# cloneofsimo/paint-with-words-sd

Hardware: AMD Instinct MI355X
Metric: 512x512 images/sec (30 steps, CFG) SD1.5+PwW (higher is better)
Workload: dtype bf16

## Files before the change

### include/pww_hip.h

```cpp
#ifndef PWW_HIP_H
#define PWW_HIP_H

#include <stddef.h>
#include <stdint.h>

#ifdef __cplusplus
extern "C" {
#endif

#define PWW_VERSION 126

#define PWW_OK 0
#define PWW_EINVAL (-22)
#define PWW_ENOTSUP (-95)
#define PWW_EHIP (-5)

#define PWW_DTYPE_F16 0
#define PWW_DTYPE_BF16 1

#define PWW_MAX_HEAD_DIM 160

typedef struct pww_attn_desc {
    int32_t dtype;
    int32_t B, H, N, M, D;
// ... 55 lines not shown
    int64_t k_stride[2];
} pww_qproj_desc_t;

int pww_qproj_stat(const void *x, const void *w, void *q, const void *k, const float *gate, const pww_qproj_desc_t *desc,
                   int32_t stat_kind, double *partials, size_t partials_bytes, void *stream);
int32_t pww_qproj_parts(const pww_qproj_desc_t *desc);

int pww_cross_attn_fwd_parts(const void *q, const void *k, const void *v, void *o, const float *bias, int32_t stat_kind,
                             float coeff_scalar, const float *gate, const pww_attn_desc_t *desc, const double *partials,
                             int32_t nparts, double *stats_out, const pww_cross_opts_t *opts, void *stream);

int pww_qk_parts(const void *q, const void *k, const float *gate, const pww_attn_desc_t *desc, int32_t stat_kind, int32_t gated_images,
                 double *partials, size_t partials_bytes, void *stream);
int32_t pww_qk_parts_count(const pww_attn_desc_t *desc);

#define PWW_LAYOUT_NCHW 0
#define PWW_LAYOUT_NHWC 1
#define PWW_ACT_NONE 0
#define PWW_ACT_SILU 1
typedef struct pww_gn_desc {
    int32_t dtype;
    int32_t layout;
    int32_t B, C, HW, G;
    float eps;
    int32_t act;
    int32_t add_stride;
    int32_t _pad;
} pww_gn_desc_t;

size_t pww_group_norm_workspace_bytes(const pww_gn_desc_t *desc);
int pww_group_norm_fwd(const void *x, const void *pre_c, const void *add_bc, const void *gamma, const void *beta, void *y,
                       const pww_gn_desc_t *desc, void *workspace, size_t workspace_bytes, void *stream);

typedef struct pww_ln_desc {
    int32_t dtype;
    int32_t C;
    int64_t rows;
    int64_t a_stride, x_stride, s_stride, y_stride;
    float eps;
    int32_t _pad;
} pww_ln_desc_t;
int pww_add_layer_norm(const void *a, const void *x, const void *gamma, const void *beta, void *s, void *y, const pww_ln_desc_t *desc, void *stream);
int pww_add_layer_norm_bias(const void *a, const void *x, const void *gamma, const void *beta, const void *post_bias, void *s, void *y,
                            const pww_ln_desc_t *desc, void *stream);
int pww_geglu(const void *h, void *y, int64_t rows, int32_t D, int64_t h_stride, int64_t y_stride, int32_t dtype, void *stream);
int pww_bias_residual(const void *r, const void *v, const void *bias, void *y, int32_t B, int32_t C, int32_t HW, int32_t layout, int32_t dtype, void *stream);

typedef struct pww_conv_desc {
    uint32_t size;
    int32_t dtype;
    int32_t B, Hin, Win, Cin, Cout;
    int32_t stride, upsample;
    int32_t tile_n, splitk;
    int32_t _pad;
} pww_conv_desc_t;
size_t pww_conv3x3_workspace_bytes(const pww_conv_desc_t *desc);
int pww_conv3x3_fwd(const void *x, const void *w, const void *bias, const void *residual, void *y, const pww_conv_desc_t *desc, void *workspace,
                    size_t workspace_bytes, void *stream);

typedef struct pww_probs_desc {
    uint32_t size;
    int32_t  images;
    int32_t  accumulate;
    float    weight;
    int64_t  out_stride[2];
} pww_probs_desc_t;

int pww_cross_attn_probs(const void *q, const void *k, const float *bias,
                         const double *stats, int32_t stat_kind, double stat_count, float coeff_scalar,
                         const float *gate, const pww_attn_desc_t *desc, const pww_cross_opts_t *opts,
                         float *out, const pww_probs_desc_t *pdesc, void *stream);

int pww_qk_reduce(const void *q, const void *k, const pww_attn_desc_t *desc,
                  double *stats, void *workspace, size_t workspace_bytes, void *stream);

typedef struct pww_region {
    uint8_t r, g, b, _pad;
    float strength;
} pww_region_t;

int pww_mask_build(const uint8_t *rgb, int32_t H, int32_t W,
                   const pww_region_t *regions, int32_t R,
                   const int32_t *col_ptr, const int32_t *col_reg, int32_t T,
                   float *out8, float *out16, float *out32, float *out64, void *stream);

int pww_mask_build_rgb(const uint8_t *rgb, int32_t H, int32_t W,
                       const pww_region_t *regions, int32_t R,
                       const int32_t *col_ptr, const int32_t *col_reg, int32_t T,
                       int32_t ratio, float *out, void *stream);

int pww_mask_build_f32(const float *masks, int32_t H, int32_t W, int32_t R,
                       const int32_t *col_ptr, const int32_t *col_reg, int32_t T,
                       int32_t ratio, float *out, void *stream);

int pww_mask_build_f32_levels(const float *masks, int32_t H, int32_t W, int32_t R, const int32_t *col_ptr, const int32_t *col_reg,
                              int32_t T, float *out8, float *out16, float *out32, float *out64, void *stream);

int pww_resize_tokens(const float *orig, int32_t H, int32_t W, int32_t T, int32_t oh, int32_t ow,
                      int32_t n_tokens, float *out, void *stream);

int pww_gauss_blur(const float *in, float *out, int32_t H, int32_t W, const float *weights, int32_t ksize,
                   double *tmp, void *stream);

int pww_inpaint_prep(const uint8_t *rgb, const uint8_t *mask, int32_t H, int32_t W, int32_t h, int32_t w,
                     float *mask_out, float *masked_image, float *mask_lat, void *stream);

int pww_cfg_combine(const void *cond, const void *uncond, float guidance, float *out,
// ... 39 lines not shown
```

### paint-with-words-sd_amd/build.py

```python
import os
import subprocess
import sys

HERE = os.path.dirname(os.path.abspath(__file__))
REPO = os.path.dirname(HERE)
CSRC = os.path.join(HERE, "csrc")
LIB = os.path.join(HERE, "pww_hip", "libpww_hip.so")
LIB_EXPERIMENTS = os.path.join(HERE, "pww_hip", "libpww_hip_experiments.so")
UNITS = [("pww_api.hip", [], ""), ("pww_attn.hip", [], ""), ("pww_cross.hip", [], ""), ("pww_cross_lean.hip", [], ""), ("pww_reduce.hip", [], ""),
         ("pww_mask.hip", [], ""), ("pww_qproj.hip", [], ""), ("pww_norm.hip", [], ""), ("pww_blocks.hip", [], ""), ("pww_conv.hip", [], ""), ("pww_probs.hip", [], ""),
         ("pww_attn_inst.hip", ["-DPWW_INST_F16"], ".f16"), ("pww_attn_inst.hip", ["-DPWW_INST_BF16"], ".bf16"),
         ("pww_cross_inst.hip", ["-DPWW_INST_F16", "-DPWW_INST_NW=2"], ".f16.nw2"), ("pww_cross_inst.hip", ["-DPWW_INST_F16", "-DPWW_INST_NW=4"], ".f16.nw4"),
         ("pww_cross_inst.hip", ["-DPWW_INST_BF16", "-DPWW_INST_NW=2"], ".bf16.nw2"), ("pww_cross_inst.hip", ["-DPWW_INST_BF16", "-DPWW_INST_NW=4"], ".bf16.nw4")]
EXPERIMENT_UNITS = [("pww_cross_out.hip", [], "")]
_ATTN_HEADERS = ["pww_tile.h", "pww_attn_core.h", "pww_cross_tile.h"]
SIDE_FLAGS = ["-fvisibility=hidden"]
SIDE_LIBS = {
    "long": ("pww_long.hip", _ATTN_HEADERS, "the long-prompt launches"),
    "scope": ("pww_scope.hip", _ATTN_HEADERS, "cross-attention with per-head / per-row score statistics"),
    "linear": ("pww_linear.hip", [], "linear layers with a bias / residual / GEGLU epilogue"),
    "regions": ("pww_regions.hip", [], "region masks and the per-pixel blend of the noise predictions"),
}
SOURCES = sorted({u[0] for u in UNITS + EXPERIMENT_UNITS})
HEADERS = ["pww_common.h", "pww_tile.h", "pww_attn_core.h", "pww_attn_kernel.h", "pww_cross_tile.h", "pww_cross_kernel.h", os.path.join(REPO, "include", "pww_hip.h")]
LIB_LONG, LIB_SCOPE, LIB_LINEAR, LIB_REGIONS = (os.path.join(HERE, "pww_hip", "libpww_hip_%s.so" % n) for n in SIDE_LIBS)
LONG_UNITS, SCOPE_UNITS, LINEAR_UNITS, REGIONS_UNITS = ([(v[0], SIDE_FLAGS, "")] for v in SIDE_LIBS.values())
HIPCC = os.environ.get("HIPCC", "/opt/rocm/bin/hipcc")
FLAGS = ["--offload-arch=gfx950", "-O3", "-std=c++17", "-fPIC", "-Wall",
         "-Wno-unused-function", "-mllvm", "-amdgpu-kernarg-preload-count=16"]


PER_FILE_FLAGS = {"pww_mask.hip": ["-ffp-contract=off"], "pww_regions.hip": ["-ffp-contract=off"]}


def _newer(target, deps):
    if not os.path.exists(target):
        return True
    t = os.path.getmtime(target)
    return any(os.path.getmtime(d) > t for d in deps)


def _deps():
    return ([os.path.join(CSRC, s) for s in SOURCES] + [h if os.path.isabs(h) else os.path.join(CSRC, h) for h in HEADERS] + [__file__])


def _build(lib, units, defines, objdir, verbose, jobs=None):
    os.makedirs(objdir, exist_ok=True)
    order = sorted(units, key=lambda u: {"pww_cross_inst.hip": 0, "pww_attn_inst.hip": 1, "pww_cross_lean.hip": 2}.get(u[0], 3))
    jobs = jobs or max(2, min(len(order), os.cpu_count() or 4, int(os.environ.get("MAX_JOBS", 16))))
    pending, running, objs = list(order), [], []
    while pending or running:
        while pending and len(running) < jobs:
            src, defs, suffix = pending.pop(0)
            o = os.path.join(objdir, src + suffix + ".o")
            objs.append(o)
            cmd = [HIPCC] + FLAGS + defines + defs + PER_FILE_FLAGS.get(src, []) + ["-c", os.path.join(CSRC, src), "-o", o]
            if verbose:
                print(" ".join(cmd))
            running.append((cmd, subprocess.Popen(cmd, stdout=subprocess.PIPE, stderr=subprocess.STDOUT, text=True)))
        cmd, p = running.pop(0)
        out, _ = p.communicate()
        if p.returncode != 0:
            for _, q in running:
                q.kill()
            raise RuntimeError("hipcc failed: %s\n%s" % (" ".join(cmd), out))
        if verbose and out.strip():
            print(out)
    subprocess.run([HIPCC, "--offload-arch=gfx950", "-shared", "-fPIC", "-s"] + sorted(objs) + ["-o", lib], check=True)
    return lib


def build_lib(force=False, verbose=False):
    if not force and not _newer(LIB, _deps()):
        return LIB
    return _build(LIB, UNITS, [], os.path.join(HERE, "build"), verbose)


# ... 49 lines not shown
```

### paint-with-words-sd_amd/csrc/pww_conv.hip

```cpp
#include "pww_common.h"

namespace pww {

namespace {

constexpr int CV_BM = 128, CV_THREADS = 256;
constexpr int CV_PF = 2;

__device__ __forceinline__ f32x4 mfma16(f16x8 a, f16x8 b, f32x4 c) { return __builtin_amdgcn_mfma_f32_16x16x32_f16(a, b, c, 0, 0, 0); }
__device__ __forceinline__ f32x4 mfma16(bf16x8 a, bf16x8 b, f32x4 c) { return __builtin_amdgcn_mfma_f32_16x16x32_bf16(a, b, c, 0, 0, 0); }

struct ConvCold {
    const void *bias, *residual;
    int nsplit, nslab;
};

__device__ __forceinline__ int xcd_remap(int orig, int nwg) {
    const int xcd = orig & 7, q = nwg >> 3, r = nwg & 7;
    return (xcd < r ? xcd * (q + 1) : r * (q + 1) + (xcd - r) * q) + (orig >> 3);
}

template <typename T>
__device__ __forceinline__ void epilogue4(const f32x4 &a, const ConvCold &cold, T *y, long off, int n) {
    typedef typename Vec<T>::v4 V4;
    V4 o;
#pragma unroll
    for (int j = 0; j < 4; ++j) o[j] = (T)a[j];
    if (cold.bias) {
        const V4 b = *reinterpret_cast<const V4 *>(reinterpret_cast<const T *>(cold.bias) + n);
#pragma unroll
        for (int j = 0; j < 4; ++j) o[j] = (T)((float)o[j] + (float)b[j]);
    }
    if (cold.residual) {
        const V4 r = *reinterpret_cast<const V4 *>(reinterpret_cast<const T *>(cold.residual) + off);
#pragma unroll
        for (int j = 0; j < 4; ++j) o[j] = (T)((float)r[j] + (float)o[j]);
    }
    *reinterpret_cast<V4 *>(y + off) = o;
}

template <typename T, int BN>
__global__ void __launch_bounds__(CV_THREADS, 2) conv3x3_kernel(const T *__restrict__ x, const T *__restrict__ w, void *__restrict__ out, int M, int N,
                                                            int Cin, int Hin, int Win, int Wo, int HWo, const ConvCold cold) {
    typedef typename Vec<T>::v8 V8;
    constexpr int BM = CV_BM, PF = CV_PF, XL = BM * 8 / CV_THREADS, WL = BN * 8 / CV_THREADS, RM = 4, RN = BN / 32;
    constexpr int XBYTES = BM * 128, STAGE = (BM + BN) * 128;
    __shared__ __attribute__((aligned(16))) char lds[2 * STAGE];

    const int geo = cold.nslab >> 24;
    const int nslab = cold.nslab & 0xffffff;
    const int stride = geo & 15, up = geo >> 4;
    const int Hv = Hin << up, Wv = Win << up;
    const int tid = threadIdx.x, lane = tid & 63, wave = tid >> 6, wm = wave >> 1, wn = wave & 1;
    const int ntm = (M + BM - 1) / BM;
    const int bid = xcd_remap(blockIdx.x, gridDim.x);
    const bool split = cold.nsplit > 1;
    const int tile = bid / cold.nsplit, ks = bid - tile * cold.nsplit;
    const int tm = tile % ntm, tn = tile / ntm;
    const int s_begin = (int)((long)ks * nslab / cold.nsplit), s_end = (int)((long)(ks + 1) * nslab / cold.nsplit);
    const int K9 = 9 * Cin;

    const int c = tid & 7;
    int pix[XL], y0[XL], x0[XL];
#pragma unroll
    for (int i = 0; i < XL; ++i) {
        int m = tm * BM + (tid >> 3) + 32 * i;
        m = m < M ? m : M - 1;
        const int b = m / HWo, rem = m - b * HWo, oy = rem / Wo, ox = rem - oy * Wo;
        pix[i] = b * Hin * Win;
        y0[i] = oy * stride - 1;
        x0[i] = ox * stride - 1;
    }
    const T *wrow = w + (long)(tn * BN + (tid >> 3)) * K9 + c * 8;
    const int swz = ((c ^ ((tid >> 3) & 7)) << 4);

    u32x4 xr[PF][XL], wr[PF][WL];
    unsigned xok[PF];
    int tap = s_begin / (Cin >> 6), ci0 = (s_begin - tap * (Cin >> 6)) << 6;
    const T *wnext = wrow + s_begin * 64;
    auto load = [&](int p) {
        const int ky = tap / 3, kx = tap - ky * 3;
        xok[p] = 0;
#pragma unroll
        for (int i = 0; i < XL; ++i) {
            const int iyv = y0[i] + ky, ixv = x0[i] + kx;
            const bool ok = (unsigned)iyv < (unsigned)Hv && (unsigned)ixv < (unsigned)Wv;
            const int iy = ok ? iyv >> up : 0, ix = ok ? ixv >> up : 0;
            xr[p][i] = *reinterpret_cast<const u32x4 *>(x + (unsigned)((pix[i] + iy * Win + ix) * Cin + ci0 + c * 8));
            xok[p] |= (unsigned)ok << i;
        }
#pragma unroll
        for (int j = 0; j < WL; ++j) wr[p][j] = *reinterpret_cast<const u32x4 *>(wnext + (long)(32 * j) * K9);
        wnext += 64;
        ci0 += 64;
        if (ci0 == Cin) { ci0 = 0; ++tap; }
    };
    auto store = [&](int p, int buf) {
        char *base = lds + buf * STAGE;
#pragma unroll
        for (int i = 0; i < XL; ++i) {
            const u32x4 z = {0u, 0u, 0u, 0u};
            *reinterpret_cast<u32x4 *>(base + ((tid >> 3) + 32 * i) * 128 + swz) = (xok[p] >> i) & 1u ? xr[p][i] : z;
        }
#pragma unroll
        for (int j = 0; j < WL; ++j) *reinterpret_cast<u32x4 *>(base + XBYTES + ((tid >> 3) + 32 * j) * 128 + swz) = wr[p][j];
    };

    f32x4 acc[RN][RM];
#pragma unroll
    for (int r = 0; r < RN; ++r)
#pragma unroll
        for (int i = 0; i < RM; ++i) acc[r][i] = f32x4{0.f, 0.f, 0.f, 0.f};

    const int fr = lane & 15, fq = lane >> 4;
    auto compute = [&](int buf) {
        const char *bx = lds + buf * STAGE, *bw = bx + XBYTES;
#pragma unroll
        for (int kk = 0; kk < 2; ++kk) {
            V8 xf[RM], wf[RN];
#pragma unroll
            for (int q = 0; q < RM; ++q) {
                const int row = wm * 64 + q * 16 + fr;
                xf[q] = *reinterpret_cast<const V8 *>(bx + row * 128 + (((kk * 4 + fq) ^ (row & 7)) << 4));
            }
#pragma unroll
            for (int r = 0; r < RN; ++r) {
                const int row = wn * (BN / 2) + r * 16 + fr;
                wf[r] = *reinterpret_cast<const V8 *>(bw + row * 128 + (((kk * 4 + fq) ^ (row & 7)) << 4));
            }
#pragma unroll
            for (int r = 0; r < RN; ++r)
#pragma unroll
                for (int q = 0; q < RM; ++q) acc[r][q] = mfma16(wf[r], xf[q], acc[r][q]);
        }
    };

    const int n = s_end - s_begin;
    load(0);
#pragma unroll
    for (int p = 1; p < PF; ++p)
        if (p < n) load(p);
    store(0, 0);
    __syncthreads();
    int i = 0;
    for (; i + 2 * PF <= n; i += PF) {
#pragma unroll
        for (int p = 0; p < PF; ++p) {
            load(p);
            compute((i + p) & 1);
            store((p + 1) % PF, (i + p + 1) & 1);
            __syncthreads();
        }
    }
#pragma unroll
    for (int t = 0; t < 2 * PF - 1; ++t) {
        if (i + t < n) {
            if (i + t + PF < n) load(t % PF);
            compute((i + t) & 1);
            if (i + t + 1 < n) store((t + 1) % PF, (i + t + 1) & 1);
            __syncthreads();
        }
    }

#pragma unroll
    for (int i = 0; i < RM; ++i) {
        const int m = tm * BM + wm * 64 + i * 16 + fr;
        if (m >= M) continue;
#pragma unroll
        for (int r = 0; r < RN; ++r) {
            const int n = tn * BN + wn * (BN / 2) + r * 16 + fq * 4;
            if (split) *reinterpret_cast<f32x4 *>(reinterpret_cast<float *>(out) + ((long)ks * M + m) * N + n) = acc[r][i];
            else epilogue4<T>(acc[r][i], cold, reinterpret_cast<T *>(out), (long)m * N + n, n);
        }
    }
}

template <typename T>
__global__ void __launch_bounds__(256) conv3x3_fold_kernel(const float *__restrict__ ws, T *__restrict__ y, long n4, int N, long MN, const ConvCold cold) {
    const long q = (long)blockIdx.x * 256 + threadIdx.x;
    if (q >= n4) return;
    const long off = q * 4;
    f32x4 a = *reinterpret_cast<const f32x4 *>(ws + off);
    for (int s = 1; s < cold.nsplit; ++s) a += *reinterpret_cast<const f32x4 *>(ws + s * MN + off);
    epilogue4<T>(a, cold, y, off, (int)(off % N));
}

struct ConvTune { int M, N, nslab, bn, nsplit; };
constexpr ConvTune CONV_TUNED[] = {
    {8192, 320, 45, 64, 3}, {8192, 320, 90, 64, 4}, {8192, 320, 135, 64, 3}, {8192, 640, 90, 128, 3},
    {2048, 320, 45, 64, 6}, {2048, 640, 45, 64, 3}, {2048, 640, 90, 128, 6}, {2048, 640, 135, 128, 6}, {2048, 640, 180, 128, 6},
    {2048, 640, 270, 128, 6}, {2048, 1280, 180, 128, 3},
    {512, 640, 90, 64, 6}, {512, 1280, 90, 128, 6}, {512, 1280, 180, 128, 12}, {512, 1280, 270, 128, 12}, {512, 1280, 360, 128, 12},
    {128, 1280, 180, 64, 12}, {128, 1280, 360, 64, 24},
    {65536, 640, 90, 128, 1}, {16384, 1280, 180, 128, 1},
    {4096, 640, 90, 128, 3}, {4096, 1280, 90, 128, 3}, {4096, 1280, 180, 128, 3}, {4096, 1280, 270, 128, 3}, {4096, 1280, 360, 128, 3},
    {1024, 1280, 180, 128, 6}, {1024, 1280, 360, 128, 6},
};

struct ConvPlan {
    int M, Ho, Wo, bn, nsplit, nslab, ntiles;
};

bool plan_conv(const pww_conv_desc_t *d, ConvPlan *p) {
    if (!d || d->size < sizeof(pww_conv_desc_t)) { set_error("conv3x3: descriptor missing or older than this library (size %u)", d ? d->size : 0u); return false; }
    const int up = d->upsample, s = d->stride;
    if ((d->dtype != PWW_DTYPE_F16 && d->dtype != PWW_DTYPE_BF16) || d->B < 1 || d->Hin < 1 || d->Win < 1 || d->Cin < 64 || d->Cin % 64 != 0
        || d->Cout < 64 || d->Cout % 64 != 0 || (s != 1 && s != 2) || (up != 0 && up != 1) || (up && s != 1) || d->Cin > 65536 || d->Cout > 65536) {
        set_error("conv3x3: unsupported (dtype %d B %d %dx%d Cin %d Cout %d stride %d upsample %d): Cin and Cout multiples of 64, stride 1 or 2, "
                  "upsample only at stride 1", d->dtype, d->B, d->Hin, d->Win, d->Cin, d->Cout, s, up);
        return false;
    }
    const int Hv = d->Hin << up, Wv = d->Win << up;
    p->Ho = (Hv - 1) / s + 1;
    p->Wo = (Wv - 1) / s + 1;
    const long M = (long)d->B * p->Ho * p->Wo;
    if ((long)d->B * d->Hin * d->Win * d->Cin >= (1L << 31) || M * d->Cout >= (1L << 31)) { set_error("conv3x3: tensor of 2^31 elements or more"); return false; }
    p->M = (int)M;
    p->nslab = 9 * d->Cin / 64;
    const ConvTune *tuned = nullptr;
    for (const ConvTune &t : CONV_TUNED)
        if (t.M == p->M && t.N == d->Cout && t.nslab == p->nslab) tuned = &t;
    p->bn = d->tile_n ? d->tile_n : tuned ? tuned->bn : (d->Cout % 128 == 0 ? 128 : 64);
    if ((p->bn != 64 && p->bn != 128) || d->Cout % p->bn != 0) { set_error("conv3x3: tile_n %d does not divide Cout %d", d->tile_n, d->Cout); return false; }
    p->ntiles = (p->M + CV_BM - 1) / CV_BM * (d->Cout / p->bn);
    int ns = d->splitk;
    if (ns <= 0 && tuned && p->bn == tuned->bn) ns = tuned->nsplit;
    if (ns <= 0) {
        ns = (480 + p->ntiles / 2) / p->ntiles;
        if (ns > p->nslab / 8) ns = p->nslab / 8;
        if (ns < 1) ns = 1;
    }
    if (ns > p->nslab || ns > 64) { set_error("conv3x3: split %d exceeds the %d K-slabs (or 64)", ns, p->nslab); return false; }
    p->nsplit = ns;
    return true;
}

template <typename T>
int conv_launch(const ConvPlan &p, const pww_conv_desc_t *d, const void *x, const void *w, const void *bias, const void *residual, void *y, void *ws,
                hipStream_t stream) {
    ConvCold cold{bias, residual, p.nsplit, p.nslab | ((d->stride | (d->upsample << 4)) << 24)};
    const T *xt = static_cast<const T *>(x), *wt = static_cast<const T *>(w);
    const int N = d->Cout, HWo = p.Ho * p.Wo;
    const dim3 grid(p.ntiles * p.nsplit), block(CV_THREADS);
    void *out = p.nsplit == 1 ? y : ws;
    if (p.bn == 128) launch_timed(conv3x3_kernel<T, 128>, grid, block, 0, stream, xt, wt, out, p.M, N, d->Cin, d->Hin, d->Win, p.Wo, HWo, cold);
    else launch_timed(conv3x3_kernel<T, 64>, grid, block, 0, stream, xt, wt, out, p.M, N, d->Cin, d->Hin, d->Win, p.Wo, HWo, cold);
    if (p.nsplit == 1) return check_hip(hipGetLastError(), "conv3x3 launch");
    const long MN = (long)p.M * N, n4 = MN / 4;
    launch_timed(conv3x3_fold_kernel<T>, dim3((unsigned)((n4 + 255) / 256)), dim3(256), 0, stream, static_cast<const float *>(ws), static_cast<T *>(y), n4,
                 N, MN, cold);
    return check_hip(hipGetLastError(), "conv3x3 fold launch");
}

bool al16(const void *a) { return (reinterpret_cast<uintptr_t>(a) & 15) == 0; }

}

size_t conv3x3_workspace_bytes(const pww_conv_desc_t *d) {
    ConvPlan p;
    if (!plan_conv(d, &p)) return 0;
    return p.nsplit > 1 ? (size_t)p.nsplit * p.M * d->Cout * sizeof(float) : 0;
}

int conv3x3_fwd(const void *x, const void *w, const void *bias, const void *residual, void *y, const pww_conv_desc_t *d, void *workspace,
                size_t workspace_bytes, hipStream_t stream) {
    ConvPlan p;
    if (!plan_conv(d, &p)) return PWW_ENOTSUP;
    if (!x || !w || !y) { set_error("conv3x3: x, w and y are required"); return PWW_EINVAL; }
    if (!al16(x) || !al16(w) || !al16(y) || (reinterpret_cast<uintptr_t>(bias) & 7) || (reinterpret_cast<uintptr_t>(residual) & 7)) {
        set_error("conv3x3: x, w, y must be 16-byte aligned, bias and residual 8-byte aligned");
        return PWW_EINVAL;
    }
    if (p.nsplit > 1 && (!workspace || !al16(workspace) || workspace_bytes < (size_t)p.nsplit * p.M * d->Cout * sizeof(float))) {
        set_error("conv3x3: split %d needs a 16-byte aligned workspace of %zu bytes (got %zu)", p.nsplit, (size_t)p.nsplit * p.M * d->Cout * sizeof(float),
                  workspace_bytes);
        return PWW_EINVAL;
    }
    if (!arch_ok()) return PWW_ENOTSUP;
    if (d->dtype == PWW_DTYPE_F16) return conv_launch<f16>(p, d, x, w, bias, residual, y, workspace, stream);
    return conv_launch<bf16>(p, d, x, w, bias, residual, y, workspace, stream);
}

}
```

### paint-with-words-sd_amd/pww_hip/_lib.py

```python
import ctypes
import os

_HERE = os.path.dirname(os.path.abspath(__file__))
LIB_PATH = os.environ.get("PWW_HIP_LIB", os.path.join(_HERE, "libpww_hip.so"))
EXPERIMENTS_LIB_PATH = os.environ.get("PWW_HIP_EXPERIMENTS_LIB", os.path.join(_HERE, "libpww_hip_experiments.so"))

LONG_LIB_PATH = os.environ.get("PWW_HIP_LONG_LIB", os.path.join(_HERE, "libpww_hip_long.so"))
SCOPE_LIB_PATH = os.environ.get("PWW_HIP_SCOPE_LIB", os.path.join(_HERE, "libpww_hip_scope.so"))
LINEAR_LIB_PATH = os.environ.get("PWW_HIP_LINEAR_LIB", os.path.join(_HERE, "libpww_hip_linear.so"))
REGIONS_LIB_PATH = os.environ.get("PWW_HIP_REGIONS_LIB", os.path.join(_HERE, "libpww_hip_regions.so"))

PWW_OK, PWW_EINVAL, PWW_ENOTSUP, PWW_EHIP = 0, -22, -95, -5
MIN_VERSION = 126
DTYPE_F16, DTYPE_BF16 = 0, 1
LAYOUT_NCHW, LAYOUT_NHWC = 0, 1
ACT_NONE, ACT_SILU = 0, 1
LINEAR_NONE, LINEAR_BIAS, LINEAR_BIAS_RESIDUAL, LINEAR_BIAS_GEGLU = 0, 1, 2, 3
MAX_HEAD_DIM = 160

EXPORTS = ("pww_version", "pww_has_experiments", "pww_last_error", "pww_device_arch", "pww_self_attn_fwd", "pww_cross_attn_fwd",
           "pww_cross_attn_fwd_stat", "pww_cross_attn_fwd_stat_ex",
           "pww_qk_reduce", "pww_mask_build", "pww_mask_build_rgb", "pww_mask_build_f32", "pww_resize_tokens", "pww_gauss_blur", "pww_inpaint_prep", "pww_cfg_combine", "pww_store_f32",
           "pww_workspace_bytes", "pww_profile_arm", "pww_profile_elapsed_us", "pww_profile_reset", "pww_debug_timeline", "pww_debug_path_counts",
           "pww_qproj_stat", "pww_qproj_parts", "pww_cross_attn_fwd_parts", "pww_mask_build_f32_levels", "pww_qk_parts", "pww_qk_parts_count",
# ... 6 lines not shown
LONG_EXPORTS = ("pww_long_version", "pww_long_last_error", "pww_long_qk_parts", "pww_long_qk_parts_count", "pww_long_cross_attn_fwd_parts",
                "pww_long_cross_attn_probs", "pww_long_profile_arm", "pww_long_profile_elapsed_us")
LONG_MIN_VERSION = 100
LONG_MIN_KEYS, LONG_MAX_KEYS = 129, 256


SCOPE_EXPORTS = ("pww_scope_version", "pww_scope_last_error", "pww_scope_head_parts_count", "pww_scope_head_parts", "pww_scope_cross_attn_fwd")
SCOPE_MIN_VERSION = 100
SCOPE_HEAD, SCOPE_ROW = 1, 2


LINEAR_EXPORTS = ("pww_linear_version", "pww_linear_last_error", "pww_linear_workspace_bytes", "pww_linear_fwd")
LINEAR_MIN_VERSION = 100


REGIONS_EXPORTS = ("pww_regions_version", "pww_regions_last_error", "pww_regions_masks", "pww_regions_combine")
REGIONS_MIN_VERSION = 100
REGIONS_MAX, REGIONS_MAX_PLANE, REGIONS_MAX_FEATHER = 8, 9216, 8.0


class AttnDesc(ctypes.Structure):
    _fields_ = [("dtype", ctypes.c_int32), ("B", ctypes.c_int32), ("H", ctypes.c_int32), ("N", ctypes.c_int32),
                ("M", ctypes.c_int32), ("D", ctypes.c_int32),
                ("q_stride", ctypes.c_int64 * 3), ("k_stride", ctypes.c_int64 * 3),
                ("v_stride", ctypes.c_int64 * 3), ("o_stride", ctypes.c_int64 * 3),
                ("scale", ctypes.c_float), ("bias_stride", ctypes.c_int64 * 4)]


class CrossOpts(ctypes.Structure):
    _fields_ = [("size", ctypes.c_uint32), ("bias_cols", ctypes.c_int32), ("coeff_scalar_dev", ctypes.c_void_p),
                ("bias_compact", ctypes.c_void_p), ("col_idx", ctypes.c_void_p), ("R", ctypes.c_int32), ("gated_images", ctypes.c_int32),
                ("compact_stride", ctypes.c_int64 * 2), ("col_idx_stride", ctypes.c_int64)]


class QprojDesc(ctypes.Structure):
    _fields_ = [("dtype", ctypes.c_int32), ("B", ctypes.c_int32), ("N", ctypes.c_int32), ("Cin", ctypes.c_int32), ("H", ctypes.c_int32),
                ("D", ctypes.c_int32), ("M", ctypes.c_int32), ("x_stride", ctypes.c_int64 * 2), ("q_stride", ctypes.c_int64 * 2),
                ("k_stride", ctypes.c_int64 * 2)]


class GnDesc(ctypes.Structure):
    _fields_ = [("dtype", ctypes.c_int32), ("layout", ctypes.c_int32), ("B", ctypes.c_int32), ("C", ctypes.c_int32), ("HW", ctypes.c_int32),
                ("G", ctypes.c_int32), ("eps", ctypes.c_float), ("act", ctypes.c_int32), ("add_stride", ctypes.c_int32), ("_pad", ctypes.c_int32)]


class LnDesc(ctypes.Structure):
    _fields_ = [("dtype", ctypes.c_int32), ("C", ctypes.c_int32), ("rows", ctypes.c_int64), ("a_stride", ctypes.c_int64), ("x_stride", ctypes.c_int64),
                ("s_stride", ctypes.c_int64), ("y_stride", ctypes.c_int64), ("eps", ctypes.c_float), ("_pad", ctypes.c_int32)]


class ConvDesc(ctypes.Structure):
    _fields_ = [("size", ctypes.c_uint32), ("dtype", ctypes.c_int32), ("B", ctypes.c_int32), ("Hin", ctypes.c_int32), ("Win", ctypes.c_int32),
                ("Cin", ctypes.c_int32), ("Cout", ctypes.c_int32), ("stride", ctypes.c_int32), ("upsample", ctypes.c_int32), ("tile_n", ctypes.c_int32),
                ("splitk", ctypes.c_int32), ("_pad", ctypes.c_int32)]


class LinearDesc(ctypes.Structure):
    _fields_ = [("size", ctypes.c_uint32), ("dtype", ctypes.c_int32), ("M", ctypes.c_int32), ("N", ctypes.c_int32), ("K", ctypes.c_int32),
                ("epilogue", ctypes.c_int32), ("x_stride", ctypes.c_int64), ("y_stride", ctypes.c_int64), ("r_stride", ctypes.c_int64),
                ("tile_n", ctypes.c_int32), ("splitk", ctypes.c_int32)]


class ProbsDesc(ctypes.Structure):
    _fields_ = [("size", ctypes.c_uint32), ("images", ctypes.c_int32), ("accumulate", ctypes.c_int32), ("weight", ctypes.c_float),
                ("out_stride", ctypes.c_int64 * 2)]


class Region(ctypes.Structure):
    _fields_ = [("r", ctypes.c_uint8), ("g", ctypes.c_uint8), ("b", ctypes.c_uint8), ("_pad", ctypes.c_uint8),
                ("strength", ctypes.c_float)]


class PwwHipError(RuntimeError):
    pass


_lib = None
_exp = None


def _bind(lib, experiments):
    vp, i32, i64, f32 = ctypes.c_void_p, ctypes.c_int32, ctypes.c_int64, ctypes.c_float
    lib.pww_version.restype = ctypes.c_int
    if lib.pww_version() // 100 != 1 or lib.pww_version() < MIN_VERSION:
        raise PwwHipError("libpww_hip ABI version %d.%02d is not 1.x >= 1.%02d (rebuild: python paint-with-words-sd_amd/build.py)"
                          % (lib.pww_version() // 100, lib.pww_version() % 100, MIN_VERSION % 100))
    lib.pww_last_error.restype = ctypes.c_char_p
    lib.pww_device_arch.argtypes = [ctypes.c_char_p, ctypes.c_size_t]
    lib.pww_self_attn_fwd.argtypes = [vp, vp, vp, vp, ctypes.POINTER(AttnDesc), vp]
    lib.pww_cross_attn_fwd.argtypes = [vp, vp, vp, vp, vp, vp, ctypes.POINTER(AttnDesc), vp]
    lib.pww_cross_attn_fwd_stat.argtypes = [vp, vp, vp, vp, vp, vp, i32, ctypes.c_double, f32, vp, ctypes.POINTER(AttnDesc), vp]
    lib.pww_cross_attn_fwd_stat_ex.argtypes = [vp, vp, vp, vp, vp, vp, i32, ctypes.c_double, f32, vp, ctypes.POINTER(AttnDesc),
                                               ctypes.POINTER(CrossOpts), vp]
    lib.pww_qproj_stat.argtypes = [vp, vp, vp, vp, vp, ctypes.POINTER(QprojDesc), i32, vp, ctypes.c_size_t, vp]
    lib.pww_qproj_stat.restype = ctypes.c_int
    lib.pww_qproj_parts.argtypes = [ctypes.POINTER(QprojDesc)]
    lib.pww_qproj_parts.restype = ctypes.c_int32
    lib.pww_cross_attn_fwd_parts.argtypes = [vp, vp, vp, vp, vp, i32, f32, vp, ctypes.POINTER(AttnDesc), vp, i32, vp, ctypes.POINTER(CrossOpts), vp]
    lib.pww_cross_attn_fwd_parts.restype = ctypes.c_int
    lib.pww_qk_parts.argtypes = [vp, vp, vp, ctypes.POINTER(AttnDesc), i32, i32, vp, ctypes.c_size_t, vp]
    lib.pww_qk_parts.restype = ctypes.c_int
    lib.pww_qk_parts_count.argtypes = [ctypes.POINTER(AttnDesc)]
    lib.pww_qk_parts_count.restype = ctypes.c_int32
    lib.pww_mask_build_f32_levels.argtypes = [vp, i32, i32, i32, vp, vp, i32, vp, vp, vp, vp, vp]
    lib.pww_mask_build_f32_levels.restype = ctypes.c_int
    lib.pww_group_norm_workspace_bytes.argtypes = [ctypes.POINTER(GnDesc)]
    lib.pww_group_norm_workspace_bytes.restype = ctypes.c_size_t
# ... 194 lines not shown
```

### paint-with-words-sd_amd/pww_hip/ops.py

```python
import ctypes

import torch

from . import _lib
from ._lib import AttnDesc, CrossOpts, ProbsDesc, QprojDesc, Region, PwwHipError

_DT = {torch.float16: _lib.DTYPE_F16, torch.bfloat16: _lib.DTYPE_BF16}


def _stream():
    return ctypes.c_void_p(torch.cuda.current_stream().cuda_stream)


def _ptr(t):
    return ctypes.c_void_p(t.data_ptr()) if t is not None else ctypes.c_void_p(0)


def _require_gpu(*tensors):
    for t in tensors:
        if t is not None and not t.is_cuda:
            raise PwwHipError("pww_hip ops need tensors on a HIP device (got %s); there is no CPU path" % t.device)


def _rows_ok(t):
# ... 862 lines not shown
        r = _rows(h, "geglu")
    if r is None:
        raise PwwHipError("geglu: the last dim must be 2 * D with D a multiple of 8 (got %d)" % h.shape[-1])
    rows, C2, hs = r
    if C2 % 16 != 0:
        raise PwwHipError("geglu: the last dim must be 2 * D with D a multiple of 8 (got %d)" % C2)
    D = C2 // 2
    y = torch.empty(h.shape[:-1] + (D,), dtype=h.dtype, device=h.device)
    with torch.cuda.device(h.device):
        _lib.check(_lib.load().pww_geglu(_ptr(h), _ptr(y), rows, D, hs, D, _DT[h.dtype], _stream()), "pww_geglu")
    return y


def bias_residual(residual, value, bias):
    _require_gpu(residual, value, bias)
    if residual.shape != value.shape or residual.dtype != value.dtype or residual.dtype not in _DT or residual.dim() != 4 or bias.dtype != residual.dtype:
        raise PwwHipError("bias_residual: two same-shape 4-d float16/bfloat16 tensors and a bias of that type are needed")
    B, C, H, W = residual.shape
    if tuple(bias.shape) != (C,):
        raise PwwHipError("bias_residual: bias must have shape (%d,), got %s" % (C, tuple(bias.shape)))
    nhwc = value.is_contiguous(memory_format=torch.channels_last) and not value.is_contiguous()
    fmt = torch.channels_last if nhwc else torch.contiguous_format
    value, residual = value.contiguous(memory_format=fmt), residual.contiguous(memory_format=fmt)
    layout = _lib.LAYOUT_NHWC if nhwc else _lib.LAYOUT_NCHW
    y = torch.empty_like(value)
    with torch.cuda.device(value.device):
        _lib.check(_lib.load().pww_bias_residual(_ptr(residual), _ptr(value), _ptr(bias.contiguous()), _ptr(y), B, C, H * W, layout, _DT[value.dtype], _stream()),
                   "pww_bias_residual")
    return y


def _khwc_weight(weight):
    if weight.is_contiguous(memory_format=torch.channels_last):
        return weight
    key = (weight.data_ptr(), weight._version, weight.dtype, weight.device)
    hit = weight.__dict__.get("_pww_khwc")
    if hit is not None and hit[0] == key:
        return hit[1]
    packed = weight.detach().permute(0, 2, 3, 1).contiguous()
    weight.__dict__["_pww_khwc"] = (key, packed)
    return packed


def conv3x3_takes(x, weight, stride=1, upsample=False):
    if not (torch.is_tensor(x) and x.is_cuda and x.dim() == 4 and x.dtype in _DT and torch.is_tensor(weight) and weight.dtype == x.dtype and weight.dim() == 4):
        return False
    B, C, H, W = x.shape
    Cout = weight.shape[0]
    return (tuple(weight.shape[1:]) == (C, 3, 3) and C % 64 == 0 and Cout % 64 == 0 and stride in (1, 2) and not (upsample and stride != 1)
            and x.is_contiguous(memory_format=torch.channels_last) and x.data_ptr() % 16 == 0
            and B * H * W * C < 2 ** 31 // 4)


def conv3x3(x, weight, bias=None, residual=None, stride=1, upsample=False, tile_n=0, splitk=0):
    _require_gpu(x, weight, bias, residual)
    if not conv3x3_takes(x, weight, stride, upsample):
        raise PwwHipError("conv3x3: needs a channels_last float16/bfloat16 x with Cin, Cout multiples of 64 and a 3 x 3 weight of its dtype")
    B, C, H, W = x.shape
    Cout = weight.shape[0]
    Hv, Wv = H << int(bool(upsample)), W << int(bool(upsample))
    Ho, Wo = (Hv - 1) // stride + 1, (Wv - 1) // stride + 1
    w = _khwc_weight(weight)
    if bias is not None and (bias.dtype != x.dtype or tuple(bias.shape) != (Cout,)):
        raise PwwHipError("conv3x3: bias must be a %s [%d]" % (x.dtype, Cout))
    if bias is not None:
        bias = bias.contiguous()
    if residual is not None:
        if tuple(residual.shape) != (B, Cout, Ho, Wo) or residual.dtype != x.dtype:
            raise PwwHipError("conv3x3: residual must be a %s %s" % (x.dtype, (B, Cout, Ho, Wo)))
        residual = residual.contiguous(memory_format=torch.channels_last)
    d = _lib.ConvDesc(ctypes.sizeof(_lib.ConvDesc), _DT[x.dtype], B, H, W, C, Cout, int(stride), int(bool(upsample)), int(tile_n), int(splitk), 0)
    lib = _lib.load()
    y = torch.empty((B, Cout, Ho, Wo), dtype=x.dtype, device=x.device, memory_format=torch.channels_last)
    nbytes = int(lib.pww_conv3x3_workspace_bytes(ctypes.byref(d)))
    ws = torch.empty(nbytes // 4, dtype=torch.float32, device=x.device) if nbytes else None
    with torch.cuda.device(x.device):
        _lib.check(lib.pww_conv3x3_fwd(_ptr(x), _ptr(w), _ptr(bias), _ptr(residual), _ptr(y), ctypes.byref(d), _ptr(ws), nbytes, _stream()), "pww_conv3x3_fwd")
    return y


def _linear_weight(weight):
    if not torch.is_tensor(weight) or weight.dim() not in (2, 4) or (weight.dim() == 4 and tuple(weight.shape[2:]) != (1, 1)):
        return None
    w = weight.detach().reshape(weight.shape[0], weight.shape[1]) if weight.dim() == 4 else weight.detach()
    return w if w.is_contiguous() and w.data_ptr() == weight.data_ptr() and w.data_ptr() % 16 == 0 else None


def linear_takes(x, weight, geglu=False, bias=None, residual=None, out=None):
    if not (torch.is_tensor(x) and x.is_cuda and x.dtype in _DT and x.dim() >= 2 and torch.is_tensor(weight) and weight.dtype == x.dtype):
        return False
    w = _linear_weight(weight)
    if w is None or x.shape[-1] != w.shape[1] or x.numel() == 0 or _rows(x, "linear") is None:
        return False
    N, K = w.shape
    rows, _, xs = _rows(x, "linear")
    if not (K % 64 == 0 and N % (128 if geglu else 64) == 0 and rows * xs < 2 ** 31 and rows * N < 2 ** 31 and N * K < 2 ** 31):
        return False
    if bias is not None and not (torch.is_tensor(bias) and bias.is_cuda and bias.dtype == x.dtype and tuple(bias.shape) == (N,) and bias.is_contiguous()
                                 and bias.data_ptr() % 8 == 0):
        return False
    shape = tuple(x.shape[:-1]) + (N // 2 if geglu else N,)
    for t in (residual, out):
        if t is not None and not (torch.is_tensor(t) and t.is_cuda and t.dtype == x.dtype and tuple(t.shape) == shape and _rows(t, "linear") is not None):
            return False
    return True


def linear(x, weight, bias=None, residual=None, geglu=False, tile_n=0, splitk=0, out=None):
    _require_gpu(x, weight, bias, residual, out)
    if not linear_takes(x, weight, geglu):
        raise PwwHipError("linear: needs a float16/bfloat16 [..., K] x with one row pitch and a dense [N, K] weight of its dtype, K and N multiples of 64%s"
                          % (" (geglu: N / 2 a multiple of 64)" if geglu else ""))
    w = _linear_weight(weight)
    N, K = w.shape
    M, _, xs = _rows(x, "linear")
    nout = N // 2 if geglu else N
    if (geglu or residual is not None) and bias is None:
        raise PwwHipError("linear: the residual and GEGLU epilogues need the bias")
    if geglu and residual is not None:
        raise PwwHipError("linear: geglu and residual exclude each other")
    if bias is not None:
        if bias.dtype != x.dtype or tuple(bias.shape) != (N,):
            raise PwwHipError("linear: bias must be a %s [%d]" % (x.dtype, N))
        bias = bias.contiguous() if bias.data_ptr() % 8 == 0 else bias.clone(memory_format=torch.contiguous_format)
# ... 24 lines not shown
```

Measured before the change: 5.136.

## Split conv3x3 K range across wave groups inside a workgroup with LDS reduction

Adds intra-workgroup K splitting (ksub) to the 3x3 conv kernel. Each 256-thread group covers a sub-range of K slabs with its own LDS stages, and the partial accumulators are summed through LDS before the epilogue. This lets the tuning table replace part of the global split-K, along with its fp32 workspace traffic and fold kernel, with on-chip reduction for small-M layers. LDS moves to dynamic allocation, and launch bounds change from 2 blocks per CU to larger blocks, which may shift register allocation and occupancy.

```diff
diff --git a/include/pww_hip.h b/include/pww_hip.h
--- a/include/pww_hip.h
+++ b/include/pww_hip.h
@@ -131,7 +131,7 @@
     int32_t B, Hin, Win, Cin, Cout;
     int32_t stride, upsample;
     int32_t tile_n, splitk;
-    int32_t _pad;
+    int32_t ksub;
 } pww_conv_desc_t;
 size_t pww_conv3x3_workspace_bytes(const pww_conv_desc_t *desc);
 int pww_conv3x3_fwd(const void *x, const void *w, const void *bias, const void *residual, void *y, const pww_conv_desc_t *desc, void *workspace,
diff --git a/paint-with-words-sd_amd/build.py b/paint-with-words-sd_amd/build.py
--- a/paint-with-words-sd_amd/build.py
+++ b/paint-with-words-sd_amd/build.py
@@ -22,7 +22,7 @@
     "regions": ("pww_regions.hip", [], "region masks and the per-pixel blend of the noise predictions"),
 }
 SOURCES = sorted({u[0] for u in UNITS + EXPERIMENT_UNITS})
-HEADERS = ["pww_common.h", "pww_tile.h", "pww_attn_core.h", "pww_attn_kernel.h", "pww_cross_tile.h", "pww_cross_kernel.h", os.path.join(REPO, "include", "pww_hip.h")]
+HEADERS = ["pww_common.h", "pww_conv_plan.h", "pww_tile.h", "pww_attn_core.h", "pww_attn_kernel.h", "pww_cross_tile.h", "pww_cross_kernel.h", os.path.join(REPO, "include", "pww_hip.h")]
 LIB_LONG, LIB_SCOPE, LIB_LINEAR, LIB_REGIONS = (os.path.join(HERE, "pww_hip", "libpww_hip_%s.so" % n) for n in SIDE_LIBS)
 LONG_UNITS, SCOPE_UNITS, LINEAR_UNITS, REGIONS_UNITS = ([(v[0], SIDE_FLAGS, "")] for v in SIDE_LIBS.values())
 HIPCC = os.environ.get("HIPCC", "/opt/rocm/bin/hipcc")
diff --git a/paint-with-words-sd_amd/csrc/pww_conv.hip b/paint-with-words-sd_amd/csrc/pww_conv.hip
--- a/paint-with-words-sd_amd/csrc/pww_conv.hip
+++ b/paint-with-words-sd_amd/csrc/pww_conv.hip
@@ -1,4 +1,7 @@
 #include "pww_common.h"
+#include "pww_conv_plan.h"
+
+#include <cstdlib>
 
 namespace pww {
 
@@ -39,25 +42,32 @@
     *reinterpret_cast<V4 *>(y + off) = o;
 }
 
+constexpr int conv_max_ksub(int bn) { return bn == 64 ? 3 : 2; }
+constexpr int conv_stage_bytes(int bn) { return (CV_BM + bn) * 128; }
+
 template <typename T, int BN>
-__global__ void __launch_bounds__(CV_THREADS, 2) conv3x3_kernel(const T *__restrict__ x, const T *__restrict__ w, void *__restrict__ out, int M, int N,
+__global__ void __launch_bounds__(CV_THREADS * conv_max_ksub(BN)) conv3x3_kernel(const T *__restrict__ x, const T *__restrict__ w, void *__restrict__ out, int M, int N,
                                                             int Cin, int Hin, int Win, int Wo, int HWo, const ConvCold cold) {
     typedef typename Vec<T>::v8 V8;
     constexpr int BM = CV_BM, PF = CV_PF, XL = BM * 8 / CV_THREADS, WL = BN * 8 / CV_THREADS, RM = 4, RN = BN / 32;
     constexpr int XBYTES = BM * 128, STAGE = (BM + BN) * 128;
-    __shared__ __attribute__((aligned(16))) char lds[2 * STAGE];
+    extern __shared__ __attribute__((aligned(16))) char conv_lds[];
 
     const int geo = cold.nslab >> 24;
     const int nslab = cold.nslab & 0xffffff;
     const int stride = geo & 15, up = geo >> 4;
     const int Hv = Hin << up, Wv = Win << up;
-    const int tid = threadIdx.x, lane = tid & 63, wave = tid >> 6, wm = wave >> 1, wn = wave & 1;
+    const int ksub = cold.nsplit >> 8, nsplit = cold.nsplit & 255;
+    const int grp = __builtin_amdgcn_readfirstlane((int)threadIdx.x >> 8);
+    char *lds = conv_lds + grp * (2 * STAGE);
+    const int tid = threadIdx.x & (CV_THREADS - 1), lane = tid & 63, wave = tid >> 6, wm = wave >> 1, wn = wave & 1;
     const int ntm = (M + BM - 1) / BM;
     const int bid = xcd_remap(blockIdx.x, gridDim.x);
-    const bool split = cold.nsplit > 1;
-    const int tile = bid / cold.nsplit, ks = bid - tile * cold.nsplit;
+    const bool split = nsplit > 1;
+    const int tile = bid / nsplit, ks = bid - tile * nsplit;
     const int tm = tile % ntm, tn = tile / ntm;
-    const int s_begin = (int)((long)ks * nslab / cold.nsplit), s_end = (int)((long)(ks + 1) * nslab / cold.nsplit);
+    int s_begin, s_end;
+    conv_slab_range(nslab, nsplit, ksub, ks, grp, &s_begin, &s_end);
     const int K9 = 9 * Cin;
 
     const int c = tid & 7;
@@ -162,6 +172,28 @@
         }
     }
 
+    if (ksub > 1) {
+        f32x4 *mine = reinterpret_cast<f32x4 *>(lds) + tid;
+        if (grp > 0) {
+#pragma unroll
+            for (int r = 0; r < RN; ++r)
+#pragma unroll
+                for (int i = 0; i < RM; ++i) mine[(r * RM + i) * CV_THREADS] = acc[r][i];
+        }
+        __syncthreads();
+        if (grp > 0) return;
+#pragma unroll
+        for (int h = 1; h < conv_max_ksub(BN); ++h) {
+            if (h < ksub) {
+                const f32x4 *theirs = mine + h * (2 * STAGE / 16);
+#pragma unroll
+                for (int r = 0; r < RN; ++r)
+#pragma unroll
+                    for (int i = 0; i < RM; ++i) acc[r][i] += theirs[(r * RM + i) * CV_THREADS];
+            }
+        }
+    }
+
 #pragma unroll
     for (int i = 0; i < RM; ++i) {
         const int m = tm * BM + wm * 64 + i * 16 + fr;
@@ -181,70 +213,104 @@
     if (q >= n4) return;
     const long off = q * 4;
     f32x4 a = *reinterpret_cast<const f32x4 *>(ws + off);
-    for (int s = 1; s < cold.nsplit; ++s) a += *reinterpret_cast<const f32x4 *>(ws + s * MN + off);
+    const int nsplit = cold.nsplit & 255;
+    for (int s = 1; s < nsplit; ++s) a += *reinterpret_cast<const f32x4 *>(ws + s * MN + off);
     epilogue4<T>(a, cold, y, off, (int)(off % N));
 }
 
-struct ConvTune { int M, N, nslab, bn, nsplit; };
+struct ConvTune { int M, N, nslab, bn, nsplit1, nsplit, ksub; };
 constexpr ConvTune CONV_TUNED[] = {
-    {8192, 320, 45, 64, 3}, {8192, 320, 90, 64, 4}, {8192, 320, 135, 64, 3}, {8192, 640, 90, 128, 3},
-    {2048, 320, 45, 64, 6}, {2048, 640, 45, 64, 3}, {2048, 640, 90, 128, 6}, {2048, 640, 135, 128, 6}, {2048, 640, 180, 128, 6},
-    {2048, 640, 270, 128, 6}, {2048, 1280, 180, 128, 3},
-    {512, 640, 90, 64, 6}, {512, 1280, 90, 128, 6}, {512, 1280, 180, 128, 12}, {512, 1280, 270, 128, 12}, {512, 1280, 360, 128, 12},
-    {128, 1280, 180, 64, 12}, {128, 1280, 360, 64, 24},
-    {65536, 640, 90, 128, 1}, {16384, 1280, 180, 128, 1},
-    {4096, 640, 90, 128, 3}, {4096, 1280, 90, 128, 3}, {4096, 1280, 180, 128, 3}, {4096, 1280, 270, 128, 3}, {4096, 1280, 360, 128, 3},
-    {1024, 1280, 180, 128, 6}, {1024, 1280, 360, 128, 6},
+    {8192, 320, 45, 64, 3, 3, 1}, {8192, 320, 90, 64, 4, 4, 1}, {8192, 320, 135, 64, 3, 3, 1}, {8192, 640, 90, 128, 3, 3, 1},
+    {2048, 320, 45, 64, 6, 3, 3}, {2048, 640, 45, 64, 3, 1, 3}, {2048, 640, 90, 128, 6, 3, 2}, {2048, 640, 135, 128, 6, 6, 1},
+    {2048, 640, 180, 128, 6, 6, 1}, {2048, 640, 270, 128, 6, 6, 1}, {2048, 1280, 180, 128, 3, 3, 1}, {512, 640, 90, 64, 6, 6, 3},
+    {512, 1280, 90, 128, 6, 6, 1}, {512, 1280, 180, 128, 12, 6, 2}, {512, 1280, 270, 128, 12, 12, 1}, {512, 1280, 360, 128, 12, 6, 2},
+    {128, 1280, 180, 64, 12, 12, 3}, {128, 1280, 360, 64, 24, 12, 3},
+    {65536, 640, 90, 128, 1, 1, 1}, {16384, 1280, 180, 128, 1, 1, 1}, {4096, 640, 90, 128, 3, 3, 1}, {4096, 1280, 90, 128, 3, 3, 1},
+    {4096, 1280, 180, 128, 3, 3, 1}, {4096, 1280, 270, 128, 3, 3, 1}, {4096, 1280, 360, 128, 3, 3, 1}, {1024, 1280, 180, 128, 6, 6, 1},
+    {1024, 1280, 360, 128, 6, 6, 1},
 };
 
 struct ConvPlan {
-    int M, Ho, Wo, bn, nsplit, nslab, ntiles;
+    int M, Ho, Wo, bn, nsplit, ksub, nslab, ntiles;
 };
 
-bool plan_conv(const pww_conv_desc_t *d, ConvPlan *p) {
-    if (!d || d->size < sizeof(pww_conv_desc_t)) { set_error("conv3x3: descriptor missing or older than this library (size %u)", d ? d->size : 0u); return false; }
+bool ksub_off() {
+    static const bool off = [] { const char *e = getenv("PWW_CONV_KSUB"); return e && e[0] == '1' && !e[1]; }();
+    return off;
+}
+
+int plan_conv(const pww_conv_desc_t *d, ConvPlan *p) {
+    if (!d || d->size < sizeof(pww_conv_desc_t)) { set_error("conv3x3: descriptor missing or older than this library (size %u)", d ? d->size : 0u); return PWW_ENOTSUP; }
     const int up = d->upsample, s = d->stride;
     if ((d->dtype != PWW_DTYPE_F16 && d->dtype != PWW_DTYPE_BF16) || d->B < 1 || d->Hin < 1 || d->Win < 1 || d->Cin < 64 || d->Cin % 64 != 0
         || d->Cout < 64 || d->Cout % 64 != 0 || (s != 1 && s != 2) || (up != 0 && up != 1) || (up && s != 1) || d->Cin > 65536 || d->Cout > 65536) {
         set_error("conv3x3: unsupported (dtype %d B %d %dx%d Cin %d Cout %d stride %d upsample %d): Cin and Cout multiples of 64, stride 1 or 2, "
                   "upsample only at stride 1", d->dtype, d->B, d->Hin, d->Win, d->Cin, d->Cout, s, up);
-        return false;
+        return PWW_ENOTSUP;
     }
     const int Hv = d->Hin << up, Wv = d->Win << up;
     p->Ho = (Hv - 1) / s + 1;
     p->Wo = (Wv - 1) / s + 1;
     const long M = (long)d->B * p->Ho * p->Wo;
-    if ((long)d->B * d->Hin * d->Win * d->Cin >= (1L << 31) || M * d->Cout >= (1L << 31)) { set_error("conv3x3: tensor of 2^31 elements or more"); return false; }
+    if ((long)d->B * d->Hin * d->Win * d->Cin >= (1L << 31) || M * d->Cout >= (1L << 31)) { set_error("conv3x3: tensor of 2^31 elements or more"); return PWW_ENOTSUP; }
     p->M = (int)M;
     p->nslab = 9 * d->Cin / 64;
     const ConvTune *tuned = nullptr;
     for (const ConvTune &t : CONV_TUNED)
         if (t.M == p->M && t.N == d->Cout && t.nslab == p->nslab) tuned = &t;
     p->bn = d->tile_n ? d->tile_n : tuned ? tuned->bn : (d->Cout % 128 == 0 ? 128 : 64);
-    if ((p->bn != 64 && p->bn != 128) || d->Cout % p->bn != 0) { set_error("conv3x3: tile_n %d does not divide Cout %d", d->tile_n, d->Cout); return false; }
+    if ((p->bn != 64 && p->bn != 128) || d->Cout % p->bn != 0) { set_error("conv3x3: tile_n %d does not divide Cout %d", d->tile_n, d->Cout); return PWW_ENOTSUP; }
     p->ntiles = (p->M + CV_BM - 1) / CV_BM * (d->Cout / p->bn);
-    int ns = d->splitk;
-    if (ns <= 0 && tuned && p->bn == tuned->bn) ns = tuned->nsplit;
-    if (ns <= 0) {
+    const int want = d->ksub;
+    if (want < 0 || want > CONV_KSUB_MAX) { set_error("conv3x3: ksub %d: 0 (the library's choice) or 1 .. %d K-groups per workgroup", want, CONV_KSUB_MAX); return PWW_EINVAL; }
+    if (want > conv_max_ksub(p->bn)) {
+        set_error("conv3x3: ksub %d does not fit the %d-wide tile (at most %d K-groups: LDS)", want, p->bn, conv_max_ksub(p->bn));
+        return PWW_EINVAL;
+    }
+    int ns = d->splitk, ksub = want ? want : 1;
+    if (ns <= 0 && tuned && p->bn == tuned->bn) {
+        if (want == 0 && !ksub_off()) { ns = tuned->nsplit; ksub = tuned->ksub; }
+        else if (want == tuned->ksub) ns = tuned->nsplit;
+        else ns = (tuned->nsplit1 + ksub / 2) / ksub;
+    } else if (ns <= 0) {
         ns = (480 + p->ntiles / 2) / p->ntiles;
         if (ns > p->nslab / 8) ns = p->nslab / 8;
-        if (ns < 1) ns = 1;
-    }
-    if (ns > p->nslab || ns > 64) { set_error("conv3x3: split %d exceeds the %d K-slabs (or 64)", ns, p->nslab); return false; }
+        ns /= ksub;
+    }
+    if (ns < 1) ns = 1;
+    if (ns > p->nslab || ns > 64) { set_error("conv3x3: split %d exceeds the %d K-slabs (or 64)", ns, p->nslab); return PWW_ENOTSUP; }
+    if (!conv_ksub_ok(p->nslab, ns, ksub)) {
+        if (want) {
+            set_error("conv3x3: ksub %d does not divide the slab count of every workgroup (%d K-slabs, split %d)", want, p->nslab, ns);
+            return PWW_EINVAL;
+        }
+        ksub = 1;
+    }
     p->nsplit = ns;
-    return true;
+    p->ksub = ksub;
+    return PWW_OK;
+}
+
+template <typename T, int BN>
+int conv_launch_bn(const ConvPlan &p, const pww_conv_desc_t *d, const T *x, const T *w, void *out, const ConvCold &cold, hipStream_t stream) {
+    constexpr size_t LDS1 = 2 * conv_stage_bytes(BN);
+    static const hipError_t attr = hipFuncSetAttribute(reinterpret_cast<const void *>(&conv3x3_kernel<T, BN>), hipFuncAttributeMaxDynamicSharedMemorySize,
+                                                       (int)(LDS1 * conv_max_ksub(BN)));
+    if (attr != hipSuccess) return check_hip(attr, "conv3x3 dynamic LDS size");
+    launch_timed(conv3x3_kernel<T, BN>, dim3(p.ntiles * p.nsplit), dim3(CV_THREADS * p.ksub), LDS1 * p.ksub, stream, x, w, out, p.M, d->Cout, d->Cin, d->Hin,
+                 d->Win, p.Wo, p.Ho * p.Wo, cold);
+    return PWW_OK;
 }
 
 template <typename T>
 int conv_launch(const ConvPlan &p, const pww_conv_desc_t *d, const void *x, const void *w, const void *bias, const void *residual, void *y, void *ws,
                 hipStream_t stream) {
-    ConvCold cold{bias, residual, p.nsplit, p.nslab | ((d->stride | (d->upsample << 4)) << 24)};
+    ConvCold cold{bias, residual, p.nsplit | (p.ksub << 8), p.nslab | ((d->stride | (d->upsample << 4)) << 24)};
     const T *xt = static_cast<const T *>(x), *wt = static_cast<const T *>(w);
-    const int N = d->Cout, HWo = p.Ho * p.Wo;
-    const dim3 grid(p.ntiles * p.nsplit), block(CV_THREADS);
+    const int N = d->Cout;
     void *out = p.nsplit == 1 ? y : ws;
-    if (p.bn == 128) launch_timed(conv3x3_kernel<T, 128>, grid, block, 0, stream, xt, wt, out, p.M, N, d->Cin, d->Hin, d->Win, p.Wo, HWo, cold);
-    else launch_timed(conv3x3_kernel<T, 64>, grid, block, 0, stream, xt, wt, out, p.M, N, d->Cin, d->Hin, d->Win, p.Wo, HWo, cold);
+    const int rc = p.bn == 128 ? conv_launch_bn<T, 128>(p, d, xt, wt, out, cold, stream) : conv_launch_bn<T, 64>(p, d, xt, wt, out, cold, stream);
+    if (rc != PWW_OK) return rc;
     if (p.nsplit == 1) return check_hip(hipGetLastError(), "conv3x3 launch");
     const long MN = (long)p.M * N, n4 = MN / 4;
     launch_timed(conv3x3_fold_kernel<T>, dim3((unsigned)((n4 + 255) / 256)), dim3(256), 0, stream, static_cast<const float *>(ws), static_cast<T *>(y), n4,
@@ -258,14 +324,15 @@
 
 size_t conv3x3_workspace_bytes(const pww_conv_desc_t *d) {
     ConvPlan p;
-    if (!plan_conv(d, &p)) return 0;
+    if (plan_conv(d, &p) != PWW_OK) return 0;
     return p.nsplit > 1 ? (size_t)p.nsplit * p.M * d->Cout * sizeof(float) : 0;
 }
 
 int conv3x3_fwd(const void *x, const void *w, const void *bias, const void *residual, void *y, const pww_conv_desc_t *d, void *workspace,
                 size_t workspace_bytes, hipStream_t stream) {
     ConvPlan p;
-    if (!plan_conv(d, &p)) return PWW_ENOTSUP;
+    const int rc = plan_conv(d, &p);
+    if (rc != PWW_OK) return rc;
     if (!x || !w || !y) { set_error("conv3x3: x, w and y are required"); return PWW_EINVAL; }
     if (!al16(x) || !al16(w) || !al16(y) || (reinterpret_cast<uintptr_t>(bias) & 7) || (reinterpret_cast<uintptr_t>(residual) & 7)) {
         set_error("conv3x3: x, w, y must be 16-byte aligned, bias and residual 8-byte aligned");
diff --git a/paint-with-words-sd_amd/csrc/pww_conv_plan.h b/paint-with-words-sd_amd/csrc/pww_conv_plan.h
--- /dev/null
+++ b/paint-with-words-sd_amd/csrc/pww_conv_plan.h
@@ -0,0 +1,29 @@
+#pragma once
+
+#if defined(__HIPCC__) || defined(__CUDACC__)
+#define PWW_CONV_HD __host__ __device__
+#else
+#define PWW_CONV_HD
+#endif
+
+namespace pww {
+
+constexpr int CONV_KSUB_MAX = 3;
+
+PWW_CONV_HD inline void conv_slab_range(int nslab, int nsplit, int ksub, int ks, int g, int *begin, int *end) {
+    const int b = (int)((long)ks * nslab / nsplit), e = (int)((long)(ks + 1) * nslab / nsplit);
+    const int n = e - b, per = ksub == 1 ? n : ksub == 2 ? n >> 1 : n / 3;
+    *begin = b + g * per;
+    *end = b + (g + 1) * per;
+}
+
+PWW_CONV_HD inline bool conv_ksub_ok(int nslab, int nsplit, int ksub) {
+    if (nsplit < 1 || nsplit > nslab || ksub < 1 || ksub > CONV_KSUB_MAX) return false;
+    for (int ks = 0; ks < nsplit; ++ks) {
+        const int n = (int)((long)(ks + 1) * nslab / nsplit) - (int)((long)ks * nslab / nsplit);
+        if (n < ksub || n % ksub != 0) return false;
+    }
+    return true;
+}
+
+}
diff --git a/paint-with-words-sd_amd/pww_hip/_lib.py b/paint-with-words-sd_amd/pww_hip/_lib.py
--- a/paint-with-words-sd_amd/pww_hip/_lib.py
+++ b/paint-with-words-sd_amd/pww_hip/_lib.py
@@ -82,7 +82,7 @@
 class ConvDesc(ctypes.Structure):
     _fields_ = [("size", ctypes.c_uint32), ("dtype", ctypes.c_int32), ("B", ctypes.c_int32), ("Hin", ctypes.c_int32), ("Win", ctypes.c_int32),
                 ("Cin", ctypes.c_int32), ("Cout", ctypes.c_int32), ("stride", ctypes.c_int32), ("upsample", ctypes.c_int32), ("tile_n", ctypes.c_int32),
-                ("splitk", ctypes.c_int32), ("_pad", ctypes.c_int32)]
+                ("splitk", ctypes.c_int32), ("ksub", ctypes.c_int32)]
 
 
 class LinearDesc(ctypes.Structure):
diff --git a/paint-with-words-sd_amd/pww_hip/ops.py b/paint-with-words-sd_amd/pww_hip/ops.py
--- a/paint-with-words-sd_amd/pww_hip/ops.py
+++ b/paint-with-words-sd_amd/pww_hip/ops.py
@@ -938,7 +938,7 @@
             and B * H * W * C < 2 ** 31 // 4)
 
 
-def conv3x3(x, weight, bias=None, residual=None, stride=1, upsample=False, tile_n=0, splitk=0):
+def conv3x3(x, weight, bias=None, residual=None, stride=1, upsample=False, tile_n=0, splitk=0, ksub=0):
     _require_gpu(x, weight, bias, residual)
     if not conv3x3_takes(x, weight, stride, upsample):
         raise PwwHipError("conv3x3: needs a channels_last float16/bfloat16 x with Cin, Cout multiples of 64 and a 3 x 3 weight of its dtype")
@@ -955,7 +955,7 @@
         if tuple(residual.shape) != (B, Cout, Ho, Wo) or residual.dtype != x.dtype:
             raise PwwHipError("conv3x3: residual must be a %s %s" % (x.dtype, (B, Cout, Ho, Wo)))
         residual = residual.contiguous(memory_format=torch.channels_last)
-    d = _lib.ConvDesc(ctypes.sizeof(_lib.ConvDesc), _DT[x.dtype], B, H, W, C, Cout, int(stride), int(bool(upsample)), int(tile_n), int(splitk), 0)
+    d = _lib.ConvDesc(ctypes.sizeof(_lib.ConvDesc), _DT[x.dtype], B, H, W, C, Cout, int(stride), int(bool(upsample)), int(tile_n), int(splitk), int(ksub))
     lib = _lib.load()
     y = torch.empty((B, Cout, Ho, Wo), dtype=x.dtype, device=x.device, memory_format=torch.channels_last)
     nbytes = int(lib.pww_conv3x3_workspace_bytes(ctypes.byref(d)))
```

New measurement: 5.153, median of 2. Within noise of the previous version (+0.3%).
